# nianticlabs/mickey

Measured on AMD Instinct MI355X. Metric: image pairs/sec (540x720), higher is better.
Workload: dtype bf16

## Files before the change

include/mickey_hip.h:

```cpp
#ifndef MICKEY_HIP_H
#define MICKEY_HIP_H

#ifdef __cplusplus
extern "C" {
#endif

typedef void* mk_stream_t;

enum { MK_OK = 0, MK_ERR_INVALID_ARGUMENT = 1, MK_ERR_LAUNCH = 2 };
enum { MK_BF16 = 0, MK_F16 = 1, MK_F32 = 2 };
enum { MK_ACT_NONE = 0, MK_ACT_RELU = 1, MK_ACT_GELU = 2 };
enum { MK_EPI_STORE = 0, MK_EPI_LS_RESIDUAL = 1, MK_EPI_QKV = 2, MK_EPI_PATCH = 3 };

int mk_version(void);
const char* mk_last_error(void);


int mk_preprocess_u8(const unsigned char* src, long long stride_img, int n, int Hs, int Ws, float* dst, int H, int W,
                     mk_stream_t stream);


int mk_gemm(const void* A, int lda, const void* W, int ldw, const float* bias, void* out, int ldc, int M, int N, int K,
            int act, int out_is_f32, int dtype, mk_stream_t stream);

int mk_gemm_grouped(const void* A, int lda, long long strideA, const void* W, int ldw, long long strideW, const float* bias,
                    long long strideBias, void* out, int ldc, long long strideOut, int groups, int M, int N, int K, int act,
                    int out_is_f32, int dtype, mk_stream_t stream);

int mk_gemm_ls_residual(const void* A, int lda, const void* W, int ldw, const float* bias, const float* gamma, float* x,
                        int ldx, int M, int N, int K, int dtype, mk_stream_t stream);

int mk_gemm_qkv(const void* A, int lda, const void* W, int ldw, const float* bias, void* q, void* k, void* vt, int nimg,
                int ntok, int ntok_pad, int heads, float qscale, int dtype, mk_stream_t stream);

int mk_gemm_patch_embed(const void* A, int lda, const void* W, int ldw, const float* bias, const float* pos, float* x,
                        int nimg, int npatch, int D, int K, int dtype, mk_stream_t stream);

int mk_im2col_patch14(const float* img, long long stride_img, long long stride_ch, int stride_row, int nimg, int gh,
                      int gw, void* out, int ldo, int dtype, mk_stream_t stream);

int mk_cls_token(const float* cls, const float* pos, float* x, int nimg, int ntok, int D, mk_stream_t stream);

int mk_gemm_ls_residual_ln(const void* A, int lda, const void* W, int ldw, const float* bias, const float* gamma, void* xh,
                           void* xl, int ldxs, float* stats, const float* shift_in, float* x_f32_out, int ldx, int M, int N,
                           int K, int dtype, mk_stream_t stream);
int mk_gemm_patch_embed_ln(const void* A, int lda, const void* W, int ldw, const float* bias, const float* pos, void* xh,
                           void* xl, float* stats, int nimg, int npatch, int D, int K, int dtype, mk_stream_t stream);
int mk_cls_token_ln(const float* cls, const float* pos, void* xh, void* xl, float* stats, int nimg, int ntok, int D, int dtype,
                    mk_stream_t stream);
int mk_recentre_split(void* xh, void* xl, float* stats, long long rows, int D, int dtype, mk_stream_t stream);
int mk_gemm_ln(const void* A, int lda, const void* W, int ldw, const float* bias, const float* colsum, const float* stats,
               float eps, float* shift_out, void* out, int ldc, int M, int N, int K, int act, int dtype, mk_stream_t stream);
int mk_gemm_qkv_ln(const void* A, int lda, const void* W, int ldw, const float* bias, const float* colsum, const float* stats,
                   float eps, float* shift_out, void* q, void* k, void* vt, int nimg, int ntok, int ntok_pad, int heads,
                   float qscale, int dtype, mk_stream_t stream);

int mk_layernorm(const float* x, int ldx, const float* w, const float* b, float eps, void* out, int ldo, int out_is_f32,
                 float* resid, int ldr, int rows_out, int D, int rows_per_img, int skip, int wgroup_rows, int bord_h,
                 int bord_w, int bord_m, int dtype, mk_stream_t stream);

int mk_layernorm_nchw(const float* x, int ldx, const float* w, const float* b, float eps, float* out, int nimg, int npix, int D,
                      int rows_per_img, int skip, int round_fp16, mk_stream_t stream);

int mk_gemm_ln128(const void* A, int lda, long long strideA, const void* W, int ldw, long long strideW, const float* ln_w,
                  const float* ln_b, float eps, float* resid, int ldr, void* out, int ldo, int groups, int M, int K, int bord_h,
                  int bord_w, int dtype, mk_stream_t stream);

int mk_layernorm_planes(const float* x, int ldx, const float* w, const float* b, float eps, void* out_hi, void* out_lo, int ldo,
                        float plane_scale, float* resid, int ldr, int rows_out, int D, int rows_per_img, int skip, int wgroup_rows,
                        int bord_h, int bord_w, int bord_m, int* sat_flag, mk_stream_t stream);

int mk_flash_attn_fwd(const void* q, const void* k, const void* vt, void* out, int ldo, int nimg, int heads, int ntok,
                      int ntok_pad, int dtype, mk_stream_t stream);


long long mk_bordered_rows(int nimg, int H, int Wd);

enum { MK_CONV_OUT_DENSE = 0, MK_CONV_OUT_BORDERED = 1, MK_CONV_OUT_F32 = 2 };
int mk_conv3x3(const void* in1, long long stride_in1, int C1, const void* in2, long long stride_in2, int C2, const void* W,
               int ldw, long long strideW, const float* bias, long long strideBias, const void* resid, long long strideResid,
               void* out, int Cout, long long strideOut, int groups, int nimg, int H, int Wd, int act, int out_kind, int dtype,
               mk_stream_t stream);

int mk_conv3x3_split(const void* in1_hi, const void* in1_lo, long long stride_in1, int C1, const void* in2_hi, const void* in2_lo,
                     long long stride_in2, int C2, const void* W, int ldw, long long strideW, const float* bias,
                     long long strideBias, void* out, void* out_lo, int Cout, long long strideOut, int groups, int nimg, int H,
                     int Wd, int act, int out_bordered, float acc_scale, float plane_scale, int* sat_flag, mk_stream_t stream);

int mk_split_planes(const float* src, long long rows, int cols, long long ld_src, float scale, void* hi, void* lo,
                    long long ld_dst, int* sat_flag, mk_stream_t stream);

int mk_gemm_grouped_split(const void* A_hi, const void* A_lo, int lda, long long strideA, const void* W, int ldw, long long strideW,
                          const float* bias, long long strideBias, void* out, void* out_lo, int ldc, long long strideOut, int groups,
                          int M, int N, int K, int act, float acc_scale, float plane_scale, int* sat_flag, mk_stream_t stream);


int mk_conv3x3_split_dscale(const void* in_hi, const void* in_lo, int C1, const void* W, int ldw, float* out, int Cout, int nimg, int H,
                            int Wd, const float* acc_scale, mk_stream_t stream);

long long mk_absmax_scale_work_floats(void);
int mk_absmax_scale(const float* x, int d0, int d1, int d2, int d3, long long s0, long long s1, long long s2, long long s3,
                    float* work, float* scale, mk_stream_t stream);

// ... 159 lines not shown
```

mickey_amd/_native.py:

```python
import ctypes
import os

import torch

from . import build as _build

MK_BF16, MK_F16, MK_F32 = 0, 1, 2
ACT_NONE, ACT_RELU, ACT_GELU = 0, 1, 2

_P, _I, _L, _F, _U = ctypes.c_void_p, ctypes.c_int, ctypes.c_longlong, ctypes.c_float, ctypes.c_ulonglong
_CODES = {"p": _P, "i": _I, "l": _L, "f": _F, "u": _U}

SIGNATURES = {
    "mk_version": ("i", ""),
    "mk_last_error": ("s", ""),
    "mk_preprocess_u8": ("i", "pliiipiip"),
    "mk_gemm": ("i", "pipippiiiiiiip"),
    "mk_gemm_grouped": ("i", "pilpilplpiliiiiiiip"),
    "mk_gemm_ls_residual": ("i", "pipipppiiiiip"),
    "mk_gemm_qkv": ("i", "pipippppiiiifip"),
    "mk_gemm_patch_embed": ("i", "pipipppiiiiip"),
    "mk_gemm_ls_residual_ln": ("i", "pipippppipppiiiiip"),
    "mk_gemm_patch_embed_ln": ("i", "pipipppppiiiiip"),
    "mk_cls_token_ln": ("i", "pppppiiiip"),
    "mk_recentre_split": ("i", "ppplilp"),
    "mk_gemm_ln": ("i", "pipipppfppiiiiiip"),
    "mk_gemm_qkv_ln": ("i", "pipipppfppppiiiifip"),
    "mk_im2col_patch14": ("i", "plliiiipiip"),
    "mk_cls_token": ("i", "pppiiip"),
    "mk_layernorm": ("i", "pippfpiipiiiiiiiiiip"),
    "mk_layernorm_nchw": ("i", "pippfpiiiiiip"),
    "mk_gemm_ln128": ("i", "pilpilppfpipiiiiiiip"),
    "mk_layernorm_planes": ("i", "pippfppifpiiiiiiiiipp"),
    "mk_flash_attn_fwd": ("i", "ppppiiiiiip"),
    "mk_bordered_rows": ("l", "iii"),
    "mk_conv3x3": ("i", "pliplipilplplpiliiiiiiip"),
    "mk_conv3x3_split": ("i", "pplipplipilplppiliiiiiiffpp"),
    "mk_conv3x3_split_dscale": ("i", "ppipipiiiipp"),
    "mk_split_planes": ("i", "plilfpplpp"),
    "mk_absmax_scale_work_floats": ("l", ""),
    "mk_absmax_scale": ("i", "piiiillllppp"),
    "mk_conv_train_lead_rows": ("l", "i"),
    "mk_conv_train_plane_rows": ("l", "iii"),
    "mk_conv_train_planes": ("i", "plllliiiipppip"),
    "mk_conv_train_weight_planes": ("i", "piiippppp"),
    "mk_conv_wgrad_work_floats": ("l", "iiiii"),
    "mk_conv_wgrad": ("i", "ppippiiiiippppp"),
    "mk_gemm_grouped_split": ("i", "ppilpilplppiliiiiiffpp"),
    "mk_posenc_add": ("i", "ppppiiiiiip"),
    "mk_linattn_work_floats": ("l", "iiii"),
    "mk_linattn_kv": ("i", "pppiiiip"),
    "mk_linattn_apply": ("i", "pppiiiiiip"),
    "mk_linattn_kv_fused": ("i", "pilpilppiiiiip"),
    "mk_linattn_apply_fused": ("i", "pilpilppilppfpiliiiiip"),
    "mk_linattn_train_work_floats": ("l", "iiii"),
    "mk_linattn_train_fwd": ("i", "pllpllpllfpppiiiip"),
    "mk_linattn_train_bwd": ("i", "pllpllpllppfpppppiiiip"),
    "mk_train_rows_per_chunk": ("i", "i"),
    "mk_train_chunks": ("i", "i"),
    "mk_train_ln_steps": ("i", "i"),
    "mk_train_linear_fwd": ("i", "pliplipppipliiip"),
    "mk_train_linear_ln128_fwd": ("i", "pliplipppfplpppip"),
    "mk_train_linear_dgrad": ("i", "pllipppiplplipliiiip"),
    "mk_train_linear_wgrad": ("i", "pllipliplipliiiip"),
    "mk_train_tail": ("i", "plilplilpp"),
    "mk_train_ln128_fwd": ("i", "pppfplpppip"),
    "mk_train_ln128_bwd": ("i", "pppppplip"),
    "mk_head_tails": ("i", "pppppppppppiiiiiiiififp"),
    "mk_dual_softmax_work_floats": ("l", "iiii"),
    "mk_dual_softmax": ("i", "ppppfifppppiiiip"),
    "mk_dual_softmax_split_work_floats": ("l", "iii"),
    "mk_dual_softmax_split": ("i", "ppppfifppppiiiip"),
    "mk_sinkhorn_work_floats": ("l", "iii"),
    "mk_sinkhorn": ("i", "ppppfippppiiiip"),
    "mk_dual_softmax_kf": ("i", "ppppfifppppiiiipip"),
    "mk_dual_softmax_split_kf": ("i", "ppppfifppppiiiipip"),
    "mk_sinkhorn_kf": ("i", "ppppfippppiiiipip"),
    "mk_mutual_nn": ("i", "ppppiiip"),
# ... 104 lines not shown
```

mickey_amd/model.py:

```python
import collections
import copy
import os

import torch
import torch.nn as nn

from . import _native, pipeline, weights
from .config import as_cfg
from .synthetic import DINO_PREFIX, DUSTBIN_KEY, VIT_ARCH, expected_keys

_LP = {"bf16": torch.bfloat16, "fp16": torch.float16, "bfloat16": torch.bfloat16, "float16": torch.float16,
       "fp32": torch.float32, "float32": torch.float32}
DINOV2_URL = "https://dl.fbaipublicfiles.com/dinov2/dinov2_vitl14/dinov2_vitl14_pretrain.pth"


def resolve_encoder_dtype(cfg):
    v = str(cfg["AMD"].get("ENCODER_DTYPE", "auto")).lower()
    if v == "auto":
        v = "fp16" if bool(cfg["MICKEY"]["DINOV2"].get("FLOAT16", True)) else "fp32"
    if v not in _LP:
        raise ValueError("AMD.ENCODER_DTYPE must be auto | bf16 | fp16 | fp32, got %r" % v)
    return _LP[v]


# ... 23 lines not shown
    return str(cfg["AMD"].get("HEADS_DTYPE", "auto")).lower() == "split"


class _SolverView:

    def __init__(self, cfg):
        P = cfg["PROCRUSTES"]
        self.it_RANSAC = P["IT_RANSAC"]
        self.it_matches = P["IT_MATCHES"]
        self.num_samples_matches = P["NUM_SAMPLED_MATCHES"]
        self.num_corr_3d_3d = P["NUM_CORR_3D_3D"]
        self.num_refinements = P["NUM_REFINEMENTS"]
        self.th_inlier = P["TH_INLIER"]
        self.th_soft_inlier = P["TH_SOFT_INLIER"]


class _MatcherView:
    def __init__(self, owner):
        self._owner = owner

    def get_matches_list(self, scores, min_conf=0.0):
        from . import ops
        scores = scores.contiguous()
        m, c = ops.mutual_nn(scores)
        outs = []
        for b in range(scores.shape[0]):
            mb = m[b, : int(c[b])].long()
            if min_conf > 0.0 and mb.numel():
                mb = mb[scores[b, mb[:, 0], mb[:, 1]].exp() > min_conf]
            outs.append(mb)
        return outs[0] if len(outs) == 1 else outs


class _ComputeMatchesView:
    def __init__(self, owner):
        self.matcher = _MatcherView(owner)
        self.extractor = owner
        self.down_factor = owner.cfg["MICKEY"]["DINOV2"]["DOWN_FACTOR"]
        self.dsc_dim = owner.cfg["MICKEY"]["DSC_HEAD"]["LAST_DIM"]


class MickeyRelativePose(nn.Module):
    def __init__(self, cfg, dinov2_weights=None):
        super().__init__()
        self.cfg = as_cfg(cfg)
        amd = self.cfg["AMD"]
        self.lp_dtype = resolve_encoder_dtype(self.cfg)
        self.heads_dtype = resolve_heads_dtype(self.cfg, self.lp_dtype)
        self.heads_split = resolve_heads_split(self.cfg)
        self.features_lp = self.heads_split and resolve_features_lp(self.cfg, self.lp_dtype)
        self.lean = bool(amd.get("LEAN", False))
        self.ln_fold = bool(amd.get("LN_FOLD", True))
        self.ln_centre = bool(amd.get("LN_CENTRE", True))
        self.seed = int(amd.get("SEED", 0))
        self.graph_mode = amd.get("GRAPH", "auto")
        self.graph_max_images = int(amd.get("GRAPH_MAX_IMAGES", 8))
        self.graph_cache_size = int(amd.get("GRAPH_CACHE", 4))
        self._graphs = collections.OrderedDict()
        self._sat_flag = None
        self._calls = 0
        self._ctr = None
        self._anchor = nn.Parameter(torch.zeros(1), requires_grad=False)
        self._sd = {}
        self._dev_weights = None
        self._ws = pipeline.Workspace()
        self.e2e_Procrustes = _SolverView(self.cfg)
        object.__setattr__(self, "compute_matches", _ComputeMatchesView(self))
        if dinov2_weights is None:
            path = amd.get("DINOV2_WEIGHTS") or os.environ.get("MICKEY_DINOV2_WEIGHTS")
            if path and str(path).lower() != "none":
                dinov2_weights = torch.load(path, map_location="cpu")
        self._dino_injected = set()
        if dinov2_weights is not None:
            for k, v in dinov2_weights.items():
                self._sd[DINO_PREFIX + k] = v.detach().cpu()
                self._dino_injected.add(DINO_PREFIX + k)
        self.eval()

    def state_dict(self, *args, **kwargs):
        return dict(self._sd)

    def load_state_dict(self, state_dict, strict=True):
        new = {k: v.detach().cpu() for k, v in state_dict.items() if torch.is_tensor(v)}
        arch = str(self.cfg["AMD"].get("VIT", "vit_large"))
        if any(k.endswith("cls_token") for k in new):
            D = [v.shape[-1] for k, v in new.items() if k.endswith("cls_token")][0]
            arch = {v[0]: k for k, v in VIT_ARCH.items()}.get(D, arch)
        expected = expected_keys(self.cfg, arch)
        if arch != "vit_large" or any(DINO_PREFIX + "blocks." in k for k in new):
            have = [int(k[len(DINO_PREFIX) + 7:].split(".")[0]) for k in new if k.startswith(DINO_PREFIX + "blocks.")]
            if have:
                depth = 1 + max(have)
                expected = {k: s for k, s in expected.items()
                            if not k.startswith(DINO_PREFIX + "blocks.") or int(k[len(DINO_PREFIX) + 7:].split(".")[0]) < depth}
        if not any("dinov2" in k for k in new) and not any("dinov2" in k for k in self._sd):
            self._fetch_dinov2()
        merged = dict(self._sd)
        merged.update(new)
        missing = [k for k in expected if k not in merged]
        unexpected = [k for k in new if k not in expected]
        bad_shape = ["%s: %s, expected %s" % (k, tuple(merged[k].shape), expected[k]) for k in expected
                     if k in merged and tuple(merged[k].shape) != expected[k] and merged[k].numel() != 1]
        if strict and (missing or unexpected or bad_shape):
            hint = ""
            if any(k.startswith(DINO_PREFIX) for k in missing):
                hint = ("\n(MicKey checkpoints are saved without the DINOv2 weights: pass dinov2_weights=, or set "
# ... 5 lines not shown
        self._sd = merged
        self._dev_weights = None
        self._graphs.clear()
        return torch.nn.modules.module._IncompatibleKeys(missing, unexpected)

    def _fetch_dinov2(self):
        if not bool(self.cfg["AMD"].get("DINOV2_HUB", True)):
            return False
        try:
            sd = torch.hub.load_state_dict_from_url(DINOV2_URL, map_location="cpu")
        except Exception as e:
            self._hub_error = "%s: %s" % (type(e).__name__, e)
            return False
        for k, v in sd.items():
            self._sd[DINO_PREFIX + k] = v.detach().cpu()
        return True

    def on_load_checkpoint(self, checkpoint):
        sd = checkpoint["state_dict"]
        if not any("dinov2" in k for k in self._sd) and not any("dinov2" in k for k in sd):
            self._fetch_dinov2()
        for k, v in self._sd.items():
            if "dinov2" in k:
                sd[k] = v

    def is_eval_model(self, is_eval):
        if not is_eval:
            raise NotImplementedError("mickey_amd implements the inference path only")

    def _apply(self, fn, *a, **k):
        self._dev_weights = None
        self._graphs = collections.OrderedDict()
        self._ctr = None
        self._sat_flag = None
        return super()._apply(fn, *a, **k)

    @property
    def device(self):
        return self._anchor.device

    def device_weights(self):
        dev = self._anchor.device
        if dev.type != "cuda":
            raise _native.MickeyHipError("MickeyRelativePose.forward needs the module on a GPU (model.cuda()); "
                                         "mickey_amd has no CPU fallback")
        if self._dev_weights is None:
            if not self._sd:
                raise RuntimeError("no weights loaded")
            fm = self.cfg["FEATURE_MATCHER"]
            if fm["TYPE"] == "DualSoftmax" and fm["DUAL_SOFTMAX"]["USE_DUSTBIN"] and DUSTBIN_KEY not in self._sd:
                raise RuntimeError("FEATURE_MATCHER.DUAL_SOFTMAX.USE_DUSTBIN is set but the checkpoint has no %s (the "
                                   "reference's strict load fails on this too)" % DUSTBIN_KEY)
            self._dev_weights = weights.prepare(self._sd, self.cfg, dev, self.lp_dtype, heads_dtype=self.heads_dtype, heads_split=self.heads_split,
                                                ln_fold=self.ln_fold, ln_centre=self.ln_centre, features_lp=self.features_lp)
        return self._dev_weights

    def _keyframe_map(self, data):
        if "keyframe_index" not in data:
            return None
        from . import ops
        B, K = int(data["image1"].shape[0]), int(data["image0"].shape[0])
        host = torch.from_numpy(ops.check_keyframe_index(data["keyframe_index"], B, K))
        kf = self._ws.get("keyframe_index", (B,), torch.int32, self._anchor.device)
        kf.copy_(host)
        return kf

    @torch.no_grad()
    def compute_correspondences(self, data, _kf=None):
        if _kf is None:
            _kf = self._keyframe_map(data)
        W = self.device_weights()
        dev = self._anchor.device
        im0 = data["image0"].to(device=dev, dtype=torch.float32)
        im1 = data["image1"].to(device=dev, dtype=torch.float32)
        B = im0.shape[0]
        same = im0.shape == im1.shape
        if _kf is not None:
            same = im0.shape[1:] == im1.shape[1:]
        rows = (B, B) if _kf is None else (B, im1.shape[0])
        im0, im1 = (t if t.stride(3) == 1 else t.contiguous() for t in (im0, im1))
        imgs = [(im0, im1)] if same else [(im0,), (im1,)]
        outs = []
        if self.heads_split and self._sat_flag is None:
            self._sat_flag = torch.zeros((1,), device=dev, dtype=torch.int32)
        self._ws.sat_flag = self._sat_flag if self.heads_split else None
        for im in imgs:
            feat, gh, gw = pipeline.encoder_forward(W, self._ws, im)
            scr, kps, depth, dsc = pipeline.heads_forward(W, self._ws, feat, sum(t.shape[0] for t in im), gh, gw, self.cfg)
            outs.append((scr, kps, depth, dsc, gh, gw))
        if same:
            scr, kps, depth, dsc, gh, gw = outs[0]
            parts = [(scr[:B], kps[:B], depth[:B], dsc[:B], gh, gw), (scr[B:], kps[B:], depth[B:], dsc[B:], gh, gw)]
        else:
            parts = outs
        for i, (scr, kps, depth, dsc, gh, gw) in enumerate(parts):
            data["kps%d_shape" % i] = [gh, gw]
            data["depth%d_map" % i] = depth.reshape(rows[i], 1, gh, gw)
            data["kps%d" % i] = kps.contiguous()
            data["depth_kp%d" % i] = depth.contiguous()
            data["scr%d" % i] = scr.contiguous()
            data["dsc%d" % i] = dsc.contiguous()
        data["down_factor"] = self.cfg["MICKEY"]["DINOV2"]["DOWN_FACTOR"]
        scores, kp, fin = pipeline.match(W, self.cfg, data["dsc0"], data["dsc1"], data["scr0"], data["scr1"], self.lean,
                                         keyframe_index=_kf)
        if scores is not None:
            data["scores"] = scores
            data["kp_scores"] = kp
# ... 135 lines not shown
```

mickey_amd/ops.py:

```python

import numpy as np
import torch


from ._native import ACT_GELU, ACT_NONE, ACT_RELU, call, dtype_code, ptr, query, stream

LOG2E = 1.4426950408889634


def _chk(t, dtype=None):
    assert t.is_cuda and t.is_contiguous(), "expected a contiguous device tensor"
    if dtype is not None:
        assert t.dtype == dtype, "expected %s, got %s" % (dtype, t.dtype)
    return t


def preprocess_u8(frames, H, W, out=None):
    assert frames.is_cuda and frames.dtype == torch.uint8 and frames.dim() == 4 and frames.shape[3] == 3 and frames.is_contiguous()
    n, Hs, Ws, _ = frames.shape
    if out is None:
        out = torch.empty((n, 3, H, W), device=frames.device, dtype=torch.float32)
    call("mk_preprocess_u8", ptr(frames), Hs * Ws * 3, n, Hs, Ws, ptr(out), H, W, stream())
    return out

# ... 5 lines not shown
def gemm(a, w, bias=None, act=ACT_NONE, out_f32=False, out=None, lda=None, K=None):
    M = a.shape[0]
    lda = a.shape[1] if lda is None else lda
    N, ldw = w.shape
    K = min(lda, ldw) if K is None else K
    if out is None:
        out = torch.empty((M, N), device=a.device, dtype=torch.float32 if out_f32 else a.dtype)
    call("mk_gemm", ptr(a), lda, ptr(w), ldw, ptr(bias), ptr(out), out.stride(0), M, N, K, act,
         int(out.dtype == torch.float32), dtype_code(a.dtype), stream())
    return out


def gemm_grouped(a, w, bias, out, groups, M, N, K, lda, ldw, ldc, stride_a, stride_w, stride_bias, stride_out, act=ACT_NONE):
    call("mk_gemm_grouped", ptr(a), lda, stride_a, ptr(w), ldw, stride_w, ptr(bias), stride_bias, ptr(out), ldc, stride_out,
         groups, M, N, K, act, int(out.dtype == torch.float32), dtype_code(a.dtype), stream())
    return out


def gemm_ls_residual(a, w, bias, gamma, x):
    M, K = a.shape
    N = w.shape[0]
    call("mk_gemm_ls_residual", ptr(a), a.stride(0), ptr(w), w.stride(0), ptr(bias), ptr(gamma), ptr(x), x.stride(0), M, N, K,
         dtype_code(a.dtype), stream())
    return x


def gemm_qkv(a, w, bias, q, k, vt, nimg, ntok, ntok_pad, heads):
    qscale = (64.0 ** -0.5) * LOG2E
    call("mk_gemm_qkv", ptr(a), a.stride(0), ptr(w), w.stride(0), ptr(bias), ptr(q), ptr(k), ptr(vt), nimg, ntok, ntok_pad,
         heads, qscale, dtype_code(a.dtype), stream())


def gemm_ls_residual_ln(a, w, bias, gamma, xh, xl, stats, x_out=None, shift=None):
    M, K = a.shape
    N = w.shape[0]
    call("mk_gemm_ls_residual_ln", ptr(a), a.stride(0), ptr(w), w.stride(0), ptr(bias), ptr(gamma), ptr(xh), ptr(xl),
         xh.stride(0), ptr(stats), ptr(shift), ptr(x_out), x_out.stride(0) if x_out is not None else N, M, N, K,
         dtype_code(a.dtype), stream())


def gemm_patch_embed_ln(a, w, bias, pos, xh, xl, stats, nimg, npatch):
    D = w.shape[0]
    call("mk_gemm_patch_embed_ln", ptr(a), a.stride(0), ptr(w), w.stride(0), ptr(bias), ptr(pos), ptr(xh), ptr(xl), ptr(stats),
         nimg, npatch, D, w.shape[1], dtype_code(a.dtype), stream())


def cls_token_ln(cls, pos, xh, xl, stats, nimg, ntok, D):
    call("mk_cls_token_ln", ptr(cls), ptr(pos), ptr(xh), ptr(xl), ptr(stats), nimg, ntok, D, dtype_code(xh.dtype), stream())


def recentre_split(xh, xl, stats):
    rows, D = xh.shape
    call("mk_recentre_split", ptr(xh), ptr(xl), ptr(stats), rows, D, dtype_code(xh.dtype), stream())


def gemm_ln(a, w, bias, colsum, stats, eps, act=ACT_NONE, out=None, shift_out=None):
    M, K = a.shape
    N = w.shape[0]
    if out is None:
        out = torch.empty((M, N), device=a.device, dtype=a.dtype)
    call("mk_gemm_ln", ptr(a), a.stride(0), ptr(w), w.stride(0), ptr(bias), ptr(colsum), ptr(stats), float(eps), ptr(shift_out),
         ptr(out), out.stride(0), M, N, K, act, dtype_code(a.dtype), stream())
    return out


def gemm_qkv_ln(a, w, bias, colsum, stats, eps, q, k, vt, nimg, ntok, ntok_pad, heads, shift_out=None):
    qscale = (64.0 ** -0.5) * LOG2E
    call("mk_gemm_qkv_ln", ptr(a), a.stride(0), ptr(w), w.stride(0), ptr(bias), ptr(colsum), ptr(stats), float(eps),
         ptr(shift_out), ptr(q), ptr(k), ptr(vt), nimg, ntok, ntok_pad, heads, qscale, dtype_code(a.dtype), stream())


def im2col_patch14(img, gh, gw, ldo, dtype, out=None):
    assert img.dtype == torch.float32 and img.stride(3) == 1
    nimg = img.shape[0]
    if out is None:
        out = torch.empty((nimg * gh * gw, ldo), device=img.device, dtype=dtype)
    assert out.shape == (nimg * gh * gw, ldo) and out.dtype == dtype and out.is_contiguous()
    call("mk_im2col_patch14", ptr(img), img.stride(0), img.stride(1), img.stride(2), nimg, gh, gw, ptr(out), ldo,
         dtype_code(dtype), stream())
    return out


def gemm_patch_embed(a, w, bias, pos, x, nimg, npatch):
    D = w.shape[0]
    call("mk_gemm_patch_embed", ptr(a), a.stride(0), ptr(w), w.stride(0), ptr(bias), ptr(pos), ptr(x), nimg, npatch, D,
         w.shape[1], dtype_code(a.dtype), stream())


def cls_token(cls, pos, x, nimg, ntok, D):
    call("mk_cls_token", ptr(cls), ptr(pos), ptr(x), nimg, ntok, D, stream())


def layernorm(x, w, b, eps, out=None, out_dtype=torch.bfloat16, resid=None, rows_out=None, rows_per_img=None, skip=0,
              ldo=None, wgroup_rows=0, ldx=None, ldr=None, bordered=None, sat=None):
    D = w.shape[-1]
    rows_in = x.numel() // x.shape[-1]
    if rows_per_img is None:
        rows_per_img = rows_in
    if rows_out is None:
        rows_out = rows_in - skip * (rows_in // rows_per_img)
    if isinstance(out, (tuple, list)):
        oh, ol = out
        assert oh.dtype == torch.float16 and (ol is None or (ol.dtype == torch.float16 and oh.stride() == ol.stride()))
        ldo = oh.stride(-2) if ldo is None else ldo
        bh, bw, bm = (bordered[1], bordered[2], bordered[0] * bordered[1] * bordered[2]) if bordered else (0, 0, 0)
        call("mk_layernorm_planes", ptr(x), x.stride(-2) if ldx is None else ldx, ptr(w), ptr(b), float(eps), ptr(oh), ptr(ol), ldo,
# ... 677 lines not shown
```

mickey_amd/pipeline.py:

```python
import torch

from . import ops
from . import weights as wts_mod


class Workspace:

    def __init__(self):
        self.bufs = {}
        self.sat_flag = None

    def get_planes(self, name, shape, device, zero=False):
        t = self.get(name, (2,) + tuple(shape), torch.float16, device, zero=zero)
        return t[0], t[1]

    def get(self, name, shape, dtype, device, zero=False):
        key = (name, tuple(shape), dtype)
        t = self.bufs.get(key)
        if t is None or t.device != device:
            t = (torch.zeros if zero else torch.empty)(tuple(shape), dtype=dtype, device=device)
            self.bufs[key] = t
        return t


def _encoder_trunk(W, ws, img):
    imgs = list(img) if isinstance(img, (list, tuple)) else [img]
    img = imgs[0]
    dev, lp = img.device, W.lp
    _, _, H, Wd = img.shape
    assert all(t.shape[1:] == img.shape[1:] for t in imgs)
    nimg = sum(t.shape[0] for t in imgs)
    gh, gw = H // 14, Wd // 14
    npatch, D, heads = gh * gw, W.D, W.heads
    ntok = npatch + 1
    pad = (ntok + 63) // 64 * 64
    M = nimg * ntok
    pos = wts_mod.interp_pos_embed(W, gh, gw, dev)
    a = ws.get("im2col", (nimg * npatch, wts_mod.PATCH_K), lp, dev)
    r0 = 0
    for t in imgs:
        ops.im2col_patch14(t, gh, gw, wts_mod.PATCH_K, lp, out=a[r0:r0 + t.shape[0] * npatch])
        r0 += t.shape[0] * npatch
    x = ws.get("x", (M, D), torch.float32, dev)
    att = ws.get("att", (M, D), lp, dev)
    hid = ws.get("hid", (M, 4 * D), lp, dev)
    q = ws.get("q", (nimg, heads, pad, 64), lp, dev, zero=True)
    k = ws.get("k", (nimg, heads, pad, 64), lp, dev, zero=True)
    vt = ws.get("vt", (nimg, heads, 64, pad), lp, dev, zero=True)
    if getattr(W, "ln_fold", False):
        xh = ws.get("xh", (M, D), lp, dev)
        xl = ws.get("xl", (M, D), lp, dev)
        st = ws.get("ln_stats", (M, D // 64, 2), torch.float32, dev)
        sh = ws.get("ln_shift", (M,), torch.float32, dev) if getattr(W, "ln_centre", True) else None
        ops.gemm_patch_embed_ln(a, W.patch_w, W.patch_b, pos, xh, xl, st, nimg, npatch)
        ops.cls_token_ln(W.cls, pos, xh, xl, st, nimg, ntok, D)
        if sh is not None:
            ops.recentre_split(xh, xl, st)
        last = len(W.blocks) - 1
        for bi, blk in enumerate(W.blocks):
            ops.gemm_qkv_ln(xh, blk.qkv_wf, blk.qkv_bf, blk.qkv_cs, st, 1e-6, q, k, vt, nimg, ntok, pad, heads, shift_out=sh)
            ops.flash_attn(q, k, vt, att, nimg, heads, ntok, pad)
            ops.gemm_ls_residual_ln(att, blk.proj_w, blk.proj_b, blk.g1, xh, xl, st, shift=sh)
            ops.gemm_ln(xh, blk.fc1_wf, blk.fc1_bf, blk.fc1_cs, st, 1e-6, act=ops.ACT_GELU, out=hid, shift_out=sh)
            ops.gemm_ls_residual_ln(hid, blk.fc2_w, blk.fc2_b, blk.g2, xh, xl, st, x_out=x if bi == last else None, shift=sh)
    else:
        ops.gemm_patch_embed(a, W.patch_w, W.patch_b, pos, x, nimg, npatch)
        ops.cls_token(W.cls, pos, x, nimg, ntok, D)
        y = ws.get("y", (M, D), lp, dev)
        for blk in W.blocks:
            ops.layernorm(x, blk.n1w, blk.n1b, 1e-6, out=y)
            ops.gemm_qkv(y, blk.qkv_w, blk.qkv_b, q, k, vt, nimg, ntok, pad, heads)
            ops.flash_attn(q, k, vt, att, nimg, heads, ntok, pad)
            ops.gemm_ls_residual(att, blk.proj_w, blk.proj_b, blk.g1, x)
            ops.layernorm(x, blk.n2w, blk.n2b, 1e-6, out=y)
            ops.gemm(y, blk.fc1_w, blk.fc1_b, act=ops.ACT_GELU, out=hid)
            ops.gemm_ls_residual(hid, blk.fc2_w, blk.fc2_b, blk.g2, x)
    return x, nimg, gh, gw


def encoder_forward(W, ws, img):
    x, nimg, gh, gw = _encoder_trunk(W, ws, img)
    dev, lp, D = x.device, W.lp, W.D
    npatch = gh * gw
    ntok = npatch + 1
    R = ops.bordered_rows(nimg, gh, gw)
    if getattr(W, "heads_split", False):
        flp = bool(getattr(W, "features_lp", False))
        feat = ws.get_planes("feat_hl%s_%d_%d_%d" % ("_lp" if flp else "", nimg, gh, gw), (R, D), dev, zero=True)
    else:
        feat = ws.get("feat_%d_%d_%d" % (nimg, gh, gw), (R, D), getattr(W, "lp_heads", lp), dev, zero=True)
    hi_only = isinstance(feat, tuple) and bool(getattr(W, "features_lp", False))
    ops.layernorm(x, W.norm_w, W.norm_b, 1e-6, out=(feat[0], None) if hi_only else feat, rows_out=nimg * npatch, rows_per_img=ntok, skip=1,
                  bordered=(nimg, gh, gw), sat=ws.sat_flag)
    return feat, gh, gw


def encoder_features(W, ws, img, round_fp16=False):
    x, nimg, gh, gw = _encoder_trunk(W, ws, img)
    npatch = gh * gw
    out = torch.empty((nimg, W.D, gh, gw), dtype=torch.float32, device=x.device)
    ops.layernorm_nchw(x, W.norm_w, W.norm_b, 1e-6, nimg, npatch, rows_per_img=npatch + 1, skip=1, round_fp16=bool(round_fp16), out=out)
    return out


def heads_forward(W, ws, feat, nimg, gh, gw, cfg):
    dev, lp = (feat[0] if isinstance(feat, tuple) else feat).device, getattr(W, "lp_heads", W.lp)
    n = gh * gw
    M = nimg * n
    G = 4
    mk = cfg["MICKEY"]
# ... 217 lines not shown
```

mickey_amd/weights.py:

```python
import math

import torch

from .synthetic import DINO_PREFIX, DUSTBIN_KEY, EXTRACTOR_PREFIX, HEADS

PATCH_K = 640


class DeviceWeights:
    pass


def _arch_from_sd(sd, prefix):
    D = sd[prefix + "cls_token"].shape[-1]
    depth = 1 + max(int(k[len(prefix) + 7:].split(".")[0]) for k in sd if k.startswith(prefix + "blocks."))
    return D, depth, D // 64


def fold_basic_block(sd, p):
    def fold(conv, bn):
        w = sd[p + conv + ".weight"].float()
        scale = sd[p + bn + ".weight"].float() / torch.sqrt(sd[p + bn + ".running_var"].float() + 1e-5)
        bias = sd[p + bn + ".bias"].float() - sd[p + bn + ".running_mean"].float() * scale
        w = (w * scale.view(-1, 1, 1, 1)).permute(0, 2, 3, 1).reshape(w.shape[0], -1)
        return w, bias
    w1, b1 = fold("conv1", "bn1")
    w2, b2 = fold("conv2", "bn2")
    sc = sd.get(p + "shortcut.0.weight")
    if sc is not None:
        w2 = torch.cat([w2, sc.float().reshape(sc.shape[0], -1)], 1)
    return w1, b1, w2, b2, sc is not None


def fold_layernorm(w, b, ln_w, ln_b, lp_dtype):
    w = w.float()
    wf = (w * ln_w.float()[None, :]).to(lp_dtype)
    return wf, wf.float().sum(1), b.float() + w @ ln_b.float()


def prepare_encoder(sd, device, lp_dtype=torch.bfloat16, prefix=DINO_PREFIX, W=None, ln_fold=True, ln_centre=True):
    W = DeviceWeights() if W is None else W
    W.lp = lp_dtype
    dev = device

    def lp(t):
        return t.to(device=dev, dtype=lp_dtype).contiguous()

    def f32(t):
        return t.to(device=dev, dtype=torch.float32).contiguous()

    p = prefix
    D, depth, heads = _arch_from_sd(sd, p)
    W.D, W.depth, W.heads = D, depth, heads
    W.ln_fold = bool(ln_fold) and lp_dtype != torch.float32 and D % 64 == 0
    W.ln_centre = bool(ln_centre)
    wp = torch.zeros((D, PATCH_K))
    wp[:, :588] = sd[p + "patch_embed.proj.weight"].float().reshape(D, 588)
    W.patch_w, W.patch_b = lp(wp), f32(sd[p + "patch_embed.proj.bias"])
    W.cls = f32(sd[p + "cls_token"].reshape(D))
    W.pos_embed = sd[p + "pos_embed"].float().cpu()
    W.blocks = []
    for i in range(depth):
        q = p + "blocks.%d." % i
        blk = DeviceWeights()
        blk.n1w, blk.n1b = f32(sd[q + "norm1.weight"]), f32(sd[q + "norm1.bias"])
        blk.qkv_w, blk.qkv_b = lp(sd[q + "attn.qkv.weight"]), f32(sd[q + "attn.qkv.bias"])
        blk.proj_w, blk.proj_b = lp(sd[q + "attn.proj.weight"]), f32(sd[q + "attn.proj.bias"])
        blk.g1 = f32(sd[q + "ls1.gamma"])
        blk.n2w, blk.n2b = f32(sd[q + "norm2.weight"]), f32(sd[q + "norm2.bias"])
        blk.fc1_w, blk.fc1_b = lp(sd[q + "mlp.fc1.weight"]), f32(sd[q + "mlp.fc1.bias"])
        blk.fc2_w, blk.fc2_b = lp(sd[q + "mlp.fc2.weight"]), f32(sd[q + "mlp.fc2.bias"])
        blk.g2 = f32(sd[q + "ls2.gamma"])
        if W.ln_fold:
            wf, cs, bf = fold_layernorm(sd[q + "attn.qkv.weight"], sd[q + "attn.qkv.bias"], sd[q + "norm1.weight"],
                                        sd[q + "norm1.bias"], lp_dtype)
            blk.qkv_wf, blk.qkv_cs, blk.qkv_bf = lp(wf), f32(cs), f32(bf)
            wf, cs, bf = fold_layernorm(sd[q + "mlp.fc1.weight"], sd[q + "mlp.fc1.bias"], sd[q + "norm2.weight"],
                                        sd[q + "norm2.bias"], lp_dtype)
            blk.fc1_wf, blk.fc1_cs, blk.fc1_bf = lp(wf), f32(cs), f32(bf)
        W.blocks.append(blk)
    W.norm_w, W.norm_b = f32(sd[p + "norm.weight"]), f32(sd[p + "norm.bias"])
    W._pos_cache = {}
    W._pe_cache = {}
    return W


def split_weight_scale(w, target=1024.0):
    m = float(w.abs().max()) if w.numel() else 0.0
    s = float(target)
    while m * s > 32768.0 and s > 2.0 ** -14:
        s *= 0.5
    return s


def split_conv_weight(w, scale=None):
    scale = split_weight_scale(w) if scale is None else scale
    K = w.shape[-1]
    assert K % 32 == 0, "split-operand weights: K must be a multiple of 32"
    ws = w.float() * scale
    hi = ws.to(torch.float16)
    lo = (ws - hi.float()).to(torch.float16)
    lead = tuple(w.shape[:-1])
    out = torch.stack([hi.reshape(lead + (K // 32, 32)), lo.reshape(lead + (K // 32, 32))], -2).reshape(lead + (2 * K,))
    assert bool(torch.isfinite(out).all()), "weights do not fit fp16 planes"
    return out


def split_conv_weight_planes(planes):
    K2 = planes.shape[-1]
    v = planes.reshape(tuple(planes.shape[:-1]) + (K2 // 64, 2, 32))
    lead = tuple(planes.shape[:-1])
    return v[..., 0, :].reshape(lead + (K2 // 2,)), v[..., 1, :].reshape(lead + (K2 // 2,))


def prepare(sd, cfg, device, lp_dtype=torch.bfloat16, heads_dtype=None, ln_fold=True, ln_centre=True, heads_split=False,
            features_lp=False):
    W = prepare_encoder(sd, device, lp_dtype, ln_fold=ln_fold, ln_centre=ln_centre)
    dev = device
    W.lp_heads = lp_dtype if heads_dtype is None else heads_dtype
    W.heads_split = bool(heads_split)
    W.features_lp = bool(features_lp) and W.heads_split
    assert not W.heads_split or W.lp_heads == torch.float32, "split-operand convs sit in the fp32 head pipeline"


    def convw(t):
        if W.heads_split:
            sc = split_weight_scale(t)
            out = split_conv_weight(t, sc).to(device=dev).contiguous()
            out.mk_scale = sc
            return out
        return t.to(device=dev, dtype=W.lp_heads).contiguous()

    def lp(t):
        return t.to(device=dev, dtype=W.lp_heads).contiguous()

    def f32(t):
        return t.to(device=dev, dtype=torch.float32).contiguous()

    e = EXTRACTOR_PREFIX
    W.rb = []
    for b in (1, 2, 3):
        folded = [fold_basic_block(sd, e + h + ".resblock%d." % b) for h in HEADS]
        assert all(f[4] for f in folded), "resblock1-3 change the channel count, so all have a 1x1 shortcut"
        blk = DeviceWeights()
        blk.w1 = convw(torch.stack([f[0] for f in folded]))
        blk.b1 = f32(torch.stack([f[1] for f in folded]))
        blk.w2 = convw(torch.stack([f[2] for f in folded]))
        blk.b2 = f32(torch.stack([f[3] for f in folded]))
        blk.cout = blk.w1.shape[1]
        blk.cin = folded[0][0].shape[1] // 9
        W.rb.append(blk)
    kp = [fold_basic_block(sd, e + h + ".resblock4.") for h in HEADS[:3]]
    W.rb4_kp = DeviceWeights()
    W.rb4_kp.w1, W.rb4_kp.b1 = convw(torch.stack([f[0] for f in kp])), f32(torch.stack([f[1] for f in kp]))
    W.rb4_kp.w2, W.rb4_kp.b2 = convw(torch.stack([f[2] for f in kp])), f32(torch.stack([f[3] for f in kp]))
    W.rb4_kp.cout = W.rb4_kp.w1.shape[1]
    W.rb4_kp.has_sc = kp[0][4]
    ds = fold_basic_block(sd, e + "dsc_head.resblock4.")
    W.rb4_dsc = DeviceWeights()
    w2d, has_sc = ds[2], ds[4]
    if W.heads_split and not has_sc:
        w2d, has_sc = torch.cat([w2d, torch.eye(w2d.shape[0])], 1), True
    W.rb4_dsc.w1, W.rb4_dsc.b1, W.rb4_dsc.w2, W.rb4_dsc.b2 = convw(ds[0]), f32(ds[1]), convw(w2d), f32(ds[3])
    W.rb4_dsc.cout = ds[0].shape[0]
    W.rb4_dsc.has_sc = has_sc
    W.att = []
    for l in range(3):
        lay = DeviceWeights()
        def stk(name):
            return torch.stack([sd[e + h + ".att_layer.layers.%d.%s" % (l, name)].float() for h in HEADS])
# ... 45 lines not shown
```

Baseline: 281.9.

## Fuse im2col, patch-embed GEMM, CLS token and recentring into one kernel

Adds a single HIP kernel that gathers 14x14 patches from the fp32 image straight into LDS, runs the patch-embedding matmul on matrix cores, adds bias and positional embedding, and mean-centres each row in-block. It writes the hi/lo split planes and LN stats directly, and dedicated blocks handle the CLS rows. This replaces four launches (im2col, patch-embed GEMM+LN, cls token, recentre_split) and removes the im2col buffer round trip through global memory. It applies only to D=1024 with LN folding and 16-bit dtypes, and its in-block reductions and fixed tiling are specialised code that needs separate validation.

```diff
diff --git a/include/mickey_hip.h b/include/mickey_hip.h
--- a/include/mickey_hip.h
+++ b/include/mickey_hip.h
@@ -49,6 +49,9 @@
 int mk_cls_token_ln(const float* cls, const float* pos, void* xh, void* xl, float* stats, int nimg, int ntok, int D, int dtype,
                     mk_stream_t stream);
 int mk_recentre_split(void* xh, void* xl, float* stats, long long rows, int D, int dtype, mk_stream_t stream);
+int mk_patch_embed_fused(const float* img, long long stride_img, long long stride_ch, int stride_row, int nimg, int gh, int gw,
+                         const void* W, int ldw, const float* bias, const float* pos, const float* cls, void* xh, void* xl,
+                         float* stats, int img0, int D, int dtype, mk_stream_t stream);
 int mk_gemm_ln(const void* A, int lda, const void* W, int ldw, const float* bias, const float* colsum, const float* stats,
                float eps, float* shift_out, void* out, int ldc, int M, int N, int K, int act, int dtype, mk_stream_t stream);
 int mk_gemm_qkv_ln(const void* A, int lda, const void* W, int ldw, const float* bias, const float* colsum, const float* stats,
diff --git a/mickey_amd/_native.py b/mickey_amd/_native.py
--- a/mickey_amd/_native.py
+++ b/mickey_amd/_native.py
@@ -24,6 +24,7 @@
     "mk_gemm_patch_embed_ln": ("i", "pipipppppiiiiip"),
     "mk_cls_token_ln": ("i", "pppppiiiip"),
     "mk_recentre_split": ("i", "ppplilp"),
+    "mk_patch_embed_fused": ("i", "plliiiipippppppiiip"),
     "mk_gemm_ln": ("i", "pipipppfppiiiiiip"),
     "mk_gemm_qkv_ln": ("i", "pipipppfppppiiiifip"),
     "mk_im2col_patch14": ("i", "plliiiipiip"),
diff --git a/mickey_amd/csrc/mk_patch_embed.hip b/mickey_amd/csrc/mk_patch_embed.hip
--- /dev/null
+++ b/mickey_amd/csrc/mk_patch_embed.hip
@@ -0,0 +1,299 @@
+#include "mk_common.hpp"
+#include "mk_gemm_common.hpp"
+
+namespace {
+using namespace mk;
+
+constexpr int PE_BM = 64;
+constexpr int PE_D = 1024;
+constexpr int PE_K = 588, PE_KP = 640;
+constexpr int PE_APITCH = PE_KP * 2 + 16;
+constexpr int PE_A_BYTES = PE_BM * PE_APITCH;
+constexpr int PE_BPITCH = 128 * 2 + 16;
+constexpr int PE_BOUNCE_WAVE = 2 * 16 * PE_BPITCH;
+constexpr int PE_PPITCH = 68;
+constexpr int PE_PART_OFF = 8 * PE_BOUNCE_WAVE;
+constexpr int PE_MEAN_OFF = PE_PART_OFF + PE_BM * PE_PPITCH * 4;
+constexpr int PE_ROWBASE_OFF = PE_MEAN_OFF + PE_BM * 4;
+constexpr int PE_XROW_OFF = PE_ROWBASE_OFF + PE_BM * 8;
+constexpr int PE_TOK_OFF = PE_XROW_OFF + PE_BM * 4;
+constexpr int PE_LDS = PE_TOK_OFF + PE_BM * 4;
+static_assert(PE_ROWBASE_OFF >= PE_A_BYTES && PE_ROWBASE_OFF % 8 == 0, "the row tables live beside the A block");
+
+template <typename T>
+__device__ __forceinline__ float split_join(float v) {
+  const T h = (T)v;
+  const T l = (T)(v - (float)h);
+  return (float)h + (float)l;
+}
+
+template <typename T>
+__device__ __forceinline__ void cls_row(const float* __restrict__ cls, const float* __restrict__ pos, T* __restrict__ xh,
+                                        T* __restrict__ xl, float* __restrict__ stats, long long row, int lane) {
+  using V4 = typename Lp<T>::V4;
+  const int quad = lane & 15, sub = lane >> 4;
+  f32x4 x[4];
+  float sum = 0.f;
+#pragma unroll
+  for (int i = 0; i < 4; ++i) {
+    const int c = (i * 4 + sub) * 64 + quad * 4;
+    const f32x4 a = *(const f32x4*)(cls + c), b = *(const f32x4*)(pos + c);
+#pragma unroll
+    for (int e = 0; e < 4; ++e) {
+      x[i][e] = split_join<T>(a[e] + b[e]);
+      sum += x[i][e];
+    }
+  }
+  const float mean = wave_sum(sum) / (float)PE_D;
+#pragma unroll
+  for (int i = 0; i < 4; ++i) {
+    const int slot = i * 4 + sub;
+    V4 oh, ol;
+#pragma unroll
+    for (int e = 0; e < 4; ++e) {
+      x[i][e] = x[i][e] - mean;
+      oh[e] = (T)x[i][e];
+      ol[e] = (T)(x[i][e] - (float)oh[e]);
+    }
+    *(V4*)(xh + row * PE_D + slot * 64 + quad * 4) = oh;
+    *(V4*)(xl + row * PE_D + slot * 64 + quad * 4) = ol;
+    float s, q;
+    gemm::quad_stats(x[i], s, q);
+    s = gemm::row16_sum(s);
+    q = gemm::row16_sum(q);
+    if (quad == 0) ((float2*)stats)[row * (PE_D / 64) + slot] = make_float2(s, q);
+  }
+}
+
+template <typename T>
+__global__ __launch_bounds__(512) void patch_embed_fused_kernel(const float* __restrict__ img, long long stride_img, long long stride_ch,
+                                                                int stride_row, int nimg, int gh, int gw, const T* __restrict__ W, int ldw,
+                                                                const float* __restrict__ bias, const float* __restrict__ pos,
+                                                                const float* __restrict__ cls, T* __restrict__ xh, T* __restrict__ xl,
+                                                                float* __restrict__ stats, int img0, int ncls_blocks) {
+  using V8 = typename Lp<T>::V8;
+  using V4 = typename Lp<T>::V4;
+  extern __shared__ __attribute__((aligned(16))) char smem[];
+  const int tid = threadIdx.x, lane = tid & 63;
+  const int wave = __builtin_amdgcn_readfirstlane(tid >> 6);
+  const int npatch = gh * gw, ntok = npatch + 1;
+  if ((int)blockIdx.x < ncls_blocks) {
+    const int im = blockIdx.x * 8 + wave;
+    if (im < nimg) cls_row<T>(cls, pos, xh, xl, stats, (long long)(img0 + im) * ntok, lane);
+    return;
+  }
+  const int mrows = nimg * npatch;
+  const int m0 = ((int)blockIdx.x - ncls_blocks) * PE_BM;
+  long long* rowbase = (long long*)(smem + PE_ROWBASE_OFF);
+  int* xrow_tab = (int*)(smem + PE_XROW_OFF);
+  int* tok_tab = (int*)(smem + PE_TOK_OFF);
+  if (tid < PE_BM) {
+    const int m = m0 + tid;
+    const int mm = m < mrows ? m : mrows - 1;
+    const int im = mm / npatch, p = mm - im * npatch;
+    const int pr = p / gw, pc = p - pr * gw;
+    rowbase[tid] = im * stride_img + (long long)(pr * 14) * stride_row + pc * 14;
+    xrow_tab[tid] = m < mrows ? (img0 + im) * ntok + 1 + p : -1;
+    tok_tab[tid] = 1 + p;
+  }
+  for (int i = tid; i < PE_BM * 26; i += 512) {
+    const int r = i / 26, j = i - r * 26;
+    *(unsigned*)(smem + r * PE_APITCH + PE_K * 2 + j * 4) = 0u;
+  }
+  __syncthreads();
+  if (tid < 448) {
+    const int r0 = tid / 14, dx0 = tid - r0 * 14, r1 = r0 + 32;
+    const float* p0 = img + rowbase[r0] + dx0;
+    const float* p1 = img + rowbase[r1] + dx0;
+    char* d0 = smem + r0 * PE_APITCH + dx0 * 2;
+    char* d1 = d0 + 32 * PE_APITCH;
+#pragma unroll 1
+    for (int ch = 0; ch < 3; ++ch) {
+      float v0[14], v1[14];
+#pragma unroll
+      for (int dy = 0; dy < 14; ++dy) {
+        v0[dy] = __builtin_nontemporal_load(p0 + ch * stride_ch + (long long)dy * stride_row);
+        v1[dy] = __builtin_nontemporal_load(p1 + ch * stride_ch + (long long)dy * stride_row);
+      }
+#pragma unroll
+      for (int dy = 0; dy < 14; ++dy) {
+        *(T*)(d0 + ch * 392 + dy * 28) = (T)v0[dy];
+        *(T*)(d1 + ch * 392 + dy * 28) = (T)v1[dy];
+      }
+    }
+  }
+  __syncthreads();
+
+  const int fr = lane & 15, fg = lane >> 4;
+  const char* wbase = (const char*)(W + (long long)(wave * 128) * ldw);
+  const unsigned wlane = (unsigned)(fr * ldw + fg * 8) * 2u;
+  const char* alane = smem + fr * PE_APITCH + fg * 16;
+  f32x4 acc[4][8];
+#pragma unroll
+  for (int mi = 0; mi < 4; ++mi)
+#pragma unroll
+    for (int ni = 0; ni < 8; ++ni) acc[mi][ni] = f32x4{0.f, 0.f, 0.f, 0.f};
+  constexpr int NKS = PE_KP / 32;
+  auto load_w = [&](V8& dst, int ks, int ni) {
+    dst = *(const V8*)(wbase + ((long long)(ni * 16) * ldw + ks * 32) * 2 + wlane);
+  };
+  auto load_x = [&](V8 (&xf)[4], int ks) {
+#pragma unroll
+    for (int mi = 0; mi < 4; ++mi) xf[mi] = *(const V8*)(alane + mi * 16 * PE_APITCH + ks * 64);
+  };
+  V8 wf[2][8], xf[2][4];
+#pragma unroll
+  for (int s = 0; s < 2; ++s)
+#pragma unroll
+    for (int ni = 0; ni < 8; ++ni) load_w(wf[s][ni], s, ni);
+  load_x(xf[0], 0);
+#pragma unroll 1
+  for (int ks = 0; ks < NKS; ks += 2) {
+#pragma unroll
+    for (int s = 0; s < 2; ++s) {
+      const int k = ks + s;
+      const int kx = k + 1 < NKS ? k + 1 : NKS - 1, kw = k + 2 < NKS ? k + 2 : NKS - 1;
+      load_x(xf[s ^ 1], kx);
+#pragma unroll
+      for (int ni = 0; ni < 8; ++ni) {
+#pragma unroll
+        for (int mi = 0; mi < 4; ++mi) acc[mi][ni] = Lp<T>::mma16(wf[s][ni], xf[s][mi], acc[mi][ni]);
+        load_w(wf[s][ni], kw, ni);
+        __builtin_amdgcn_sched_barrier(0);
+      }
+    }
+  }
+
+#pragma unroll
+  for (int mi = 0; mi < 4; ++mi) {
+    const float* prow = pos + (long long)tok_tab[mi * 16 + fr] * PE_D + wave * 128 + fg * 4;
+#pragma unroll
+    for (int ni = 0; ni < 8; ++ni) {
+      f32x4 v = acc[mi][ni] + *(const f32x4*)(bias + wave * 128 + ni * 16 + fg * 4);
+      v += *(const f32x4*)(prow + ni * 16);
+#pragma unroll
+      for (int e = 0; e < 4; ++e) acc[mi][ni][e] = split_join<T>(v[e]);
+    }
+  }
+  __syncthreads();
+  float* part = (float*)(smem + PE_PART_OFF);
+  float* smean = (float*)(smem + PE_MEAN_OFF);
+#pragma unroll
+  for (int t = 0; t < 4; ++t) {
+    if ((wave >> 1) == t) {
+#pragma unroll
+      for (int mi = 0; mi < 4; ++mi)
+#pragma unroll
+        for (int ni = 0; ni < 8; ++ni) {
+          float* pp = part + (mi * 16 + fr) * PE_PPITCH + (2 * (wave & 1) + (ni >> 2)) * 16 + (ni & 3) * 4 + fg;
+          float s = t == 0 ? 0.f : *pp;
+          s += acc[mi][ni][0];
+          s += acc[mi][ni][1];
+          s += acc[mi][ni][2];
+          s += acc[mi][ni][3];
+          *pp = s;
+        }
+    }
+    __syncthreads();
+  }
+#pragma unroll
+  for (int i = 0; i < 8; ++i) {
+    const int r = wave * 8 + i;
+    const float s = wave_sum(part[r * PE_PPITCH + lane]);
+    if (lane == 0) smean[r] = s / (float)PE_D;
+  }
+  __syncthreads();
+  char* bh = smem + wave * PE_BOUNCE_WAVE;
+  char* bl = bh + 16 * PE_BPITCH;
+#pragma unroll
+  for (int mi = 0; mi < 4; ++mi) {
+    const float mean = smean[mi * 16 + fr];
+    float s4[8], q4[8];
+#pragma unroll
+    for (int ni = 0; ni < 8; ++ni) {
+      f32x4 c;
+      V4 oh, ol;
+#pragma unroll
+      for (int e = 0; e < 4; ++e) {
+        c[e] = acc[mi][ni][e] - mean;
+        oh[e] = (T)c[e];
+        ol[e] = (T)(c[e] - (float)oh[e]);
+      }
+      gemm::quad_stats(c, s4[ni], q4[ni]);
+      *(V4*)(bh + fr * PE_BPITCH + (ni * 16 + fg * 4) * 2) = oh;
+      *(V4*)(bl + fr * PE_BPITCH + (ni * 16 + fg * 4) * 2) = ol;
+    }
+#pragma unroll
+    for (int ni = 0; ni < 8; ++ni) {
+      s4[ni] += __shfl_xor(s4[ni], 16, 64);
+      q4[ni] += __shfl_xor(q4[ni], 16, 64);
+      s4[ni] += __shfl_xor(s4[ni], 32, 64);
+      q4[ni] += __shfl_xor(q4[ni], 32, 64);
+    }
+    const int xr = xrow_tab[mi * 16 + fr];
+    if (fg == 0 && xr >= 0) {
+#pragma unroll
+      for (int hh = 0; hh < 2; ++hh)
+        ((float2*)stats)[(long long)xr * (PE_D / 64) + 2 * wave + hh] =
+            make_float2((s4[hh * 4] + s4[hh * 4 + 1]) + (s4[hh * 4 + 2] + s4[hh * 4 + 3]),
+                        (q4[hh * 4] + q4[hh * 4 + 1]) + (q4[hh * 4 + 2] + q4[hh * 4 + 3]));
+    }
+#pragma unroll
+    for (int i = 0; i < 4; ++i) {
+      const int rr = i * 4 + fg, cc = fr;
+      const V8 vh = *(const V8*)(bh + rr * PE_BPITCH + cc * 16), vl = *(const V8*)(bl + rr * PE_BPITCH + cc * 16);
+      const int xo = xrow_tab[mi * 16 + rr];
+      if (xo >= 0) {
+        const long long o = (long long)xo * PE_D + wave * 128 + cc * 8;
+        *(V8*)(xh + o) = vh;
+        *(V8*)(xl + o) = vl;
+      }
+    }
+  }
+}
+
+template <typename T>
+int launch_patch_embed(const float* img, long long stride_img, long long stride_ch, int stride_row, int nimg, int gh, int gw,
+                       const void* W, int ldw, const float* bias, const float* pos, const float* cls, void* xh, void* xl, float* stats,
+                       int img0, hipStream_t st) {
+  static bool attr_done = false;
+  if (!attr_done) {
+    hipError_t e = hipFuncSetAttribute((const void*)patch_embed_fused_kernel<T>, hipFuncAttributeMaxDynamicSharedMemorySize, PE_LDS);
+    if (e != hipSuccess) {
+      mk_set_error("mk_patch_embed_fused: cannot reserve %d B of LDS: %s", PE_LDS, hipGetErrorString(e));
+      return MK_ERR_LAUNCH;
+    }
+    attr_done = true;
+  }
+  const int ncls = (nimg + 7) / 8;
+  const int nblk = (nimg * gh * gw + PE_BM - 1) / PE_BM;
+  hipLaunchKernelGGL((patch_embed_fused_kernel<T>), dim3(ncls + nblk), dim3(512), PE_LDS, st, img, stride_img, stride_ch, stride_row, nimg,
+                     gh, gw, (const T*)W, ldw, bias, pos, cls, (T*)xh, (T*)xl, stats, img0, ncls);
+  MK_CHECK_LAUNCH();
+  return MK_OK;
+}
+
+}
+
+extern "C" {
+
+int mk_patch_embed_fused(const float* img, long long stride_img, long long stride_ch, int stride_row, int nimg, int gh, int gw,
+                         const void* W, int ldw, const float* bias, const float* pos, const float* cls, void* xh, void* xl,
+                         float* stats, int img0, int D, int dtype, mk_stream_t stream) {
+  MK_CHECK_ARG(img && W && bias && pos && cls && xh && xl && stats, "mk_patch_embed_fused: null pointer");
+  MK_CHECK_ARG(dtype == MK_BF16 || dtype == MK_F16, "mk_patch_embed_fused: 16-bit dtypes only");
+  MK_CHECK_ARG(D == PE_D, "mk_patch_embed_fused: D=%d (built for %d; other widths take the separate launches)", D, PE_D);
+  MK_CHECK_ARG(nimg > 0 && gh > 0 && gw > 0 && img0 >= 0 && stride_row >= gw * 14, "mk_patch_embed_fused: bad geometry");
+  MK_CHECK_ARG(ldw >= PE_KP && ldw % 8 == 0, "mk_patch_embed_fused: ldw=%d must be >= %d and a multiple of 8", ldw, PE_KP);
+  MK_CHECK_ARG((((uintptr_t)W | (uintptr_t)bias | (uintptr_t)pos | (uintptr_t)cls | (uintptr_t)xh | (uintptr_t)xl) & 15) == 0 &&
+                   ((uintptr_t)stats & 7) == 0 && ((uintptr_t)img & 3) == 0,
+               "mk_patch_embed_fused: W / bias / pos / cls / xh / xl must be 16-byte aligned");
+  MK_CHECK_ARG(((long long)img0 + nimg) * ((long long)gh * gw + 1) < (1ll << 31) - PE_BM, "mk_patch_embed_fused: too many token rows");
+  if (dtype == MK_BF16)
+    return launch_patch_embed<__bf16>(img, stride_img, stride_ch, stride_row, nimg, gh, gw, W, ldw, bias, pos, cls, xh, xl, stats, img0,
+                                      (hipStream_t)stream);
+  return launch_patch_embed<_Float16>(img, stride_img, stride_ch, stride_row, nimg, gh, gw, W, ldw, bias, pos, cls, xh, xl, stats, img0,
+                                      (hipStream_t)stream);
+}
+
+}
diff --git a/mickey_amd/model.py b/mickey_amd/model.py
--- a/mickey_amd/model.py
+++ b/mickey_amd/model.py
@@ -99,6 +99,7 @@
         self.lean = bool(amd.get("LEAN", False))
         self.ln_fold = bool(amd.get("LN_FOLD", True))
         self.ln_centre = bool(amd.get("LN_CENTRE", True))
+        self.patch_fused = bool(amd.get("PATCH_FUSED", True))
         self.seed = int(amd.get("SEED", 0))
         self.graph_mode = amd.get("GRAPH", "auto")
         self.graph_max_images = int(amd.get("GRAPH_MAX_IMAGES", 8))
@@ -210,7 +211,8 @@
                 raise RuntimeError("FEATURE_MATCHER.DUAL_SOFTMAX.USE_DUSTBIN is set but the checkpoint has no %s (the "
                                    "reference's strict load fails on this too)" % DUSTBIN_KEY)
             self._dev_weights = weights.prepare(self._sd, self.cfg, dev, self.lp_dtype, heads_dtype=self.heads_dtype, heads_split=self.heads_split,
-                                                ln_fold=self.ln_fold, ln_centre=self.ln_centre, features_lp=self.features_lp)
+                                                ln_fold=self.ln_fold, ln_centre=self.ln_centre, features_lp=self.features_lp,
+                                                patch_fused=self.patch_fused)
         return self._dev_weights
 
     def _keyframe_map(self, data):
diff --git a/mickey_amd/ops.py b/mickey_amd/ops.py
--- a/mickey_amd/ops.py
+++ b/mickey_amd/ops.py
@@ -81,6 +81,18 @@
 def recentre_split(xh, xl, stats):
     rows, D = xh.shape
     call("mk_recentre_split", ptr(xh), ptr(xl), ptr(stats), rows, D, dtype_code(xh.dtype), stream())
+
+
+def patch_embed_fused(img, w, bias, pos, cls, xh, xl, stats, img0=0):
+    assert img.dtype == torch.float32 and img.dim() == 4 and img.shape[1] == 3 and img.stride(3) == 1
+    n, _, H, Wd = img.shape
+    gh, gw = H // 14, Wd // 14
+    ntok, D = gh * gw + 1, w.shape[0]
+    _chk(xh), _chk(xl, xh.dtype), _chk(stats, torch.float32), _chk(pos, torch.float32), _chk(w, xh.dtype)
+    assert xh.shape == xl.shape and xh.shape[1] == D and tuple(stats.shape) == (xh.shape[0], D // 64, 2)
+    assert tuple(pos.shape) == (ntok, D) and img0 >= 0 and (img0 + n) * ntok <= xh.shape[0]
+    call("mk_patch_embed_fused", ptr(img), img.stride(0), img.stride(1), img.stride(2), n, gh, gw, ptr(w), w.stride(0), ptr(bias),
+         ptr(pos), ptr(cls), ptr(xh), ptr(xl), ptr(stats), img0, D, dtype_code(xh.dtype), stream())
 
 
 def gemm_ln(a, w, bias, colsum, stats, eps, act=ACT_NONE, out=None, shift_out=None):
diff --git a/mickey_amd/pipeline.py b/mickey_amd/pipeline.py
--- a/mickey_amd/pipeline.py
+++ b/mickey_amd/pipeline.py
@@ -36,11 +36,14 @@
     pad = (ntok + 63) // 64 * 64
     M = nimg * ntok
     pos = wts_mod.interp_pos_embed(W, gh, gw, dev)
-    a = ws.get("im2col", (nimg * npatch, wts_mod.PATCH_K), lp, dev)
-    r0 = 0
-    for t in imgs:
-        ops.im2col_patch14(t, gh, gw, wts_mod.PATCH_K, lp, out=a[r0:r0 + t.shape[0] * npatch])
-        r0 += t.shape[0] * npatch
+    fused = (getattr(W, "patch_fused", True) and getattr(W, "ln_fold", False) and getattr(W, "ln_centre", True)
+             and D == 1024 and lp != torch.float32)
+    if not fused:
+        a = ws.get("im2col", (nimg * npatch, wts_mod.PATCH_K), lp, dev)
+        r0 = 0
+        for t in imgs:
+            ops.im2col_patch14(t, gh, gw, wts_mod.PATCH_K, lp, out=a[r0:r0 + t.shape[0] * npatch])
+            r0 += t.shape[0] * npatch
     x = ws.get("x", (M, D), torch.float32, dev)
     att = ws.get("att", (M, D), lp, dev)
     hid = ws.get("hid", (M, 4 * D), lp, dev)
@@ -52,10 +55,16 @@
         xl = ws.get("xl", (M, D), lp, dev)
         st = ws.get("ln_stats", (M, D // 64, 2), torch.float32, dev)
         sh = ws.get("ln_shift", (M,), torch.float32, dev) if getattr(W, "ln_centre", True) else None
-        ops.gemm_patch_embed_ln(a, W.patch_w, W.patch_b, pos, xh, xl, st, nimg, npatch)
-        ops.cls_token_ln(W.cls, pos, xh, xl, st, nimg, ntok, D)
-        if sh is not None:
-            ops.recentre_split(xh, xl, st)
+        if fused:
+            i0 = 0
+            for t in imgs:
+                ops.patch_embed_fused(t, W.patch_w, W.patch_b, pos, W.cls, xh, xl, st, img0=i0)
+                i0 += t.shape[0]
+        else:
+            ops.gemm_patch_embed_ln(a, W.patch_w, W.patch_b, pos, xh, xl, st, nimg, npatch)
+            ops.cls_token_ln(W.cls, pos, xh, xl, st, nimg, ntok, D)
+            if sh is not None:
+                ops.recentre_split(xh, xl, st)
         last = len(W.blocks) - 1
         for bi, blk in enumerate(W.blocks):
             ops.gemm_qkv_ln(xh, blk.qkv_wf, blk.qkv_bf, blk.qkv_cs, st, 1e-6, q, k, vt, nimg, ntok, pad, heads, shift_out=sh)
diff --git a/mickey_amd/weights.py b/mickey_amd/weights.py
--- a/mickey_amd/weights.py
+++ b/mickey_amd/weights.py
@@ -38,7 +38,7 @@
     return wf, wf.float().sum(1), b.float() + w @ ln_b.float()
 
 
-def prepare_encoder(sd, device, lp_dtype=torch.bfloat16, prefix=DINO_PREFIX, W=None, ln_fold=True, ln_centre=True):
+def prepare_encoder(sd, device, lp_dtype=torch.bfloat16, prefix=DINO_PREFIX, W=None, ln_fold=True, ln_centre=True, patch_fused=True):
     W = DeviceWeights() if W is None else W
     W.lp = lp_dtype
     dev = device
@@ -54,6 +54,7 @@
     W.D, W.depth, W.heads = D, depth, heads
     W.ln_fold = bool(ln_fold) and lp_dtype != torch.float32 and D % 64 == 0
     W.ln_centre = bool(ln_centre)
+    W.patch_fused = bool(patch_fused)
     wp = torch.zeros((D, PATCH_K))
     wp[:, :588] = sd[p + "patch_embed.proj.weight"].float().reshape(D, 588)
     W.patch_w, W.patch_b = lp(wp), f32(sd[p + "patch_embed.proj.bias"])
@@ -114,8 +115,8 @@
 
 
 def prepare(sd, cfg, device, lp_dtype=torch.bfloat16, heads_dtype=None, ln_fold=True, ln_centre=True, heads_split=False,
-            features_lp=False):
-    W = prepare_encoder(sd, device, lp_dtype, ln_fold=ln_fold, ln_centre=ln_centre)
+            features_lp=False, patch_fused=True):
+    W = prepare_encoder(sd, device, lp_dtype, ln_fold=ln_fold, ln_centre=ln_centre, patch_fused=patch_fused)
     dev = device
     W.lp_heads = lp_dtype if heads_dtype is None else heads_dtype
     W.heads_split = bool(heads_split)
```

After: 283.0 (median of 6 runs). Within noise of the previous version (+0.4%).
